# lbcb-sci/herro

Measured on NVIDIA H100. Metric: corrected_bases_per_sec, higher is better.
Workload: dtype u8 pileup/consensus + f32 forward

## Files before the change

### herro_b200/csrc/gemm_tc.cu

```cuda
#include <cstdio>
#include <cuda.h>
#include <cuda_bf16.h>

#include "common.cuh"
#include "forward.h"

namespace hb {

namespace {

constexpr int BM = 128, BN = 128, BK = 64, STAGES = 3;
constexpr int STAGE_BYTES = (2 * BM + 2 * BN) * 128;
constexpr int C_THREADS = 256, G_THREADS = 288, G_PROD_WARP = 8;

__device__ __forceinline__ uint32_t smem_u32(const void* p) { return (uint32_t)__cvta_generic_to_shared(p); }

__device__ __forceinline__ void mbar_init(uint64_t* bar, uint32_t count) {
    asm volatile("mbarrier.init.shared::cta.b64 [%0], %1;" ::"r"(smem_u32(bar)), "r"(count));
}
__device__ __forceinline__ void mbar_arrive(uint64_t* bar) {
    asm volatile("{\n\t.reg .b64 st;\n\tmbarrier.arrive.shared::cta.b64 st, [%0];\n\t}" ::"r"(smem_u32(bar)) : "memory");
}
__device__ __forceinline__ void mbar_wait(uint64_t* bar, uint32_t parity) {
    asm volatile(
// ... 141 lines not shown
}
__device__ __forceinline__ void frag_store_f32(const float (&a)[64], float* base, size_t ld, size_t row0, int c0, int fc) {
#pragma unroll
    for (int j = 0; j < 16; j++) {
        *(float2*)(base + row0 * ld + c0 + 8 * j + fc) = make_float2(a[4 * j], a[4 * j + 1]);
        *(float2*)(base + (row0 + 8) * ld + c0 + 8 * j + fc) = make_float2(a[4 * j + 2], a[4 * j + 3]);
    }
}
__device__ __forceinline__ void frag_store_split(const float (&a)[64], __nv_bfloat16* hi, __nv_bfloat16* lo, size_t ld, size_t row0, int c0,
                                                 int fc) {
#pragma unroll
    for (int j = 0; j < 16; j++) {
        uint32_t h, l;
        const size_t o0 = row0 * ld + c0 + 8 * j + fc, o1 = (row0 + 8) * ld + c0 + 8 * j + fc;
        split2(a[4 * j], a[4 * j + 1], h, l);
        *(uint32_t*)(hi + o0) = h; *(uint32_t*)(lo + o0) = l;
        split2(a[4 * j + 2], a[4 * j + 3], h, l);
        *(uint32_t*)(hi + o1) = h; *(uint32_t*)(lo + o1) = l;
    }
}
__device__ __forceinline__ void frag_store_tile(const float (&a)[64], uint8_t* tile, int r, int fc, const float* gam = nullptr,
                                                const float* bet = nullptr, const float* ln = nullptr) {
#pragma unroll
    for (int j = 0; j < 16; j++)
#pragma unroll
        for (int hf = 0; hf < 2; hf++) {
            const int rr = r + 8 * hf, c = 8 * j + fc;
            float x = a[4 * j + 2 * hf], y = a[4 * j + 2 * hf + 1];
            if (gam) {
                x = (x - ln[2 * hf]) * ln[2 * hf + 1] * gam[c] + bet[c];
                y = (y - ln[2 * hf]) * ln[2 * hf + 1] * gam[c + 1] + bet[c + 1];
            }
            uint32_t h, l;
            split2(x, y, h, l);
            const uint32_t off = (uint32_t)(j >> 3) * (2 * BM * 128) + (uint32_t)rr * 128u + (uint32_t)((((j & 7) ^ (rr & 7)) << 4) + fc * 2);
            *(uint32_t*)(tile + off) = h;
            *(uint32_t*)(tile + off + BM * 128) = l;
        }
}

}

__global__ void __launch_bounds__(G_THREADS, 1) k_gemm_ws(GemmArgs g, const __grid_constant__ CUtensorMap tmAhi,
                                                         const __grid_constant__ CUtensorMap tmAlo, const __grid_constant__ CUtensorMap tmWhi,
                                                         const __grid_constant__ CUtensorMap tmWlo) {
    extern __shared__ uint8_t smem_dyn[];
    uint8_t* smem = smem_dyn + ((1024u - (smem_u32(smem_dyn) & 1023u)) & 1023u);
    __shared__ uint64_t full_bar[STAGES], empty_bar[STAGES];
    __shared__ __align__(16) float s_lng[BN], s_lnb[BN];

    const int tid = threadIdx.x, warp = tid >> 5, lane = tid & 31;
    if (tid == 0) {
        for (int s = 0; s < STAGES; s++) { mbar_init(&full_bar[s], 1); mbar_init(&empty_bar[s], C_THREADS); }
        asm volatile("fence.mbarrier_init.release.cluster;" ::: "memory");
    }
    if (g.mode == GEMM_OUT_F32_RES_LN && tid < BN) { s_lng[tid] = g.ln_g[tid]; s_lnb[tid] = g.ln_b[tid]; }
    __syncthreads();

    const uint32_t n_items = g.m_tiles * g.n_chunks;
    const uint32_t kbs = g.k_blocks;

    if (warp == G_PROD_WARP) {
        if (lane == 0) {
            uint32_t it_stage = 0;
            for (uint32_t item = blockIdx.x; item < n_items; item += gridDim.x) {
                const int m0 = (int)((item / g.n_chunks) * BM), n0 = (int)((item % g.n_chunks) * BN);
                for (uint32_t kb = 0; kb < kbs; kb++, it_stage++) {
                    const uint32_t s = it_stage % STAGES, ph = (it_stage / STAGES) & 1;
                    mbar_wait(&empty_bar[s], ph ^ 1);
                    const uint32_t sb = smem_u32(smem + (size_t)s * STAGE_BYTES);
                    const int k0 = (int)(kb * BK);
                    mbar_arrive_expect_tx(&full_bar[s], STAGE_BYTES);
                    tma_load_2d(sb, &tmAhi, &full_bar[s], k0, m0);
                    tma_load_2d(sb + BM * 128, &tmAlo, &full_bar[s], k0, m0);
                    tma_load_2d(sb + 2 * BM * 128, &tmWhi, &full_bar[s], k0, n0);
                    tma_load_2d(sb + 2 * BM * 128 + BN * 128, &tmWlo, &full_bar[s], k0, n0);
                }
            }
        }
        return;
    }
    const int wg = warp >> 2;
    const int fr = wg * 64 + (warp & 3) * 16 + (lane >> 2), fc = (lane & 3) * 2;
    uint32_t it_stage = 0;
    float acc[64];
    for (uint32_t item = blockIdx.x; item < n_items; item += gridDim.x) {
        const uint32_t m0 = (item / g.n_chunks) * BM, n0 = (item % g.n_chunks) * BN;
        uint32_t prev = 0;
        for (uint32_t kb = 0; kb < kbs; kb++, it_stage++) {
            const uint32_t s = it_stage % STAGES, ph = (it_stage / STAGES) & 1;
            mbar_wait(&full_bar[s], ph);
            const uint32_t sb = smem_u32(smem + (size_t)s * STAGE_BYTES);
            mma_kblock(acc, sb + wg * 64 * 128, sb + BM * 128 + wg * 64 * 128, sb + 2 * BM * 128, sb + 2 * BM * 128 + BN * 128, kb == 0);
            if (kb > 0) {
                wg_wait<1>();
                mbar_arrive(&empty_bar[prev]);
            }
            prev = s;
        }
        wg_wait<0>();
        acc_fence(acc);
        mbar_arrive(&empty_bar[prev]);
        const size_t row0 = (size_t)m0 + fr;
        if (g.mode == GEMM_OUT_F32_RES_LN) {
#pragma unroll
            for (int j = 0; j < 16; j++) {
                const int c = 8 * j + fc;
                const float2 bv = *(const float2*)(g.bias + c);
                const float2 x0 = *(const float2*)(g.res + row0 * g.ldc + c), x1 = *(const float2*)(g.res + (row0 + 8) * g.ldc + c);
                acc[4 * j] = acc[4 * j] + bv.x + x0.x; acc[4 * j + 1] = acc[4 * j + 1] + bv.y + x0.y;
                acc[4 * j + 2] = acc[4 * j + 2] + bv.x + x1.x; acc[4 * j + 3] = acc[4 * j + 3] + bv.y + x1.y;
            }
            frag_store_f32(acc, g.out, g.ldc, row0, 0, fc);
            frag_layernorm(acc, s_lng, s_lnb, fc);
            frag_store_split(acc, g.out_hi, g.out_lo, g.ldo, row0, 0, fc);
            continue;
        }
#pragma unroll
        for (int j = 0; j < 16; j++) {
            const int c = (int)n0 + 8 * j + fc;
            const float2 bv = *(const float2*)(g.bias + c);
            acc[4 * j] += bv.x; acc[4 * j + 1] += bv.y; acc[4 * j + 2] += bv.x; acc[4 * j + 3] += bv.y;
            if (g.mode == GEMM_OUT_F32_RES) {
                const float2 x0 = *(const float2*)(g.res + row0 * g.ldc + c), x1 = *(const float2*)(g.res + (row0 + 8) * g.ldc + c);
                acc[4 * j] += x0.x; acc[4 * j + 1] += x0.y; acc[4 * j + 2] += x1.x; acc[4 * j + 3] += x1.y;
            } else if (g.mode == GEMM_OUT_F32_RELU || g.mode == GEMM_OUT_SPLIT_RELU) {
#pragma unroll
                for (int e = 0; e < 4; e++) acc[4 * j + e] = fmaxf(acc[4 * j + e], 0.f);
            }
        }
        if (g.mode == GEMM_OUT_SPLIT_RELU) frag_store_split(acc, g.out_hi, g.out_lo, g.ldo, row0, (int)n0, fc);
        else frag_store_f32(acc, g.out, g.ldc, row0, (int)n0, fc);
    }
}

constexpr int FFN_RING_BYTES = 2 * BN * 128;
constexpr int FFN_A_BYTES = 2 * 2 * BM * 128;
constexpr int FFN_STAGES = 4;
constexpr int FFN_THREADS = 384, FFN_PROD_WARP = 8, FFN_PROD_REGS = 24, FFN_CONS_REGS = 240;

template <int N>
__device__ __forceinline__ void ffn_retire(uint64_t* empty_bar, uint32_t it_stage) {
    wg_wait<N>();
    mbar_arrive(&empty_bar[(it_stage - 1 - N) % FFN_STAGES]);
    if constexpr (N > 0) ffn_retire<N - 1>(empty_bar, it_stage);
}

template <bool FUSE_O>
__global__ void __launch_bounds__(FFN_THREADS, 1) k_ffn_ws(FfnArgs g, const __grid_constant__ CUtensorMap tmHhi,
                                                        const __grid_constant__ CUtensorMap tmHlo, const __grid_constant__ CUtensorMap tmW1hi,
                                                        const __grid_constant__ CUtensorMap tmW1lo, const __grid_constant__ CUtensorMap tmW2hi,
                                                        const __grid_constant__ CUtensorMap tmW2lo, const __grid_constant__ CUtensorMap tmWohi,
                                                        const __grid_constant__ CUtensorMap tmWolo) {
    extern __shared__ uint8_t smem_dyn[];
    uint8_t* smem = smem_dyn + ((1024u - (smem_u32(smem_dyn) & 1023u)) & 1023u);
    uint8_t* sA1 = smem;
    uint8_t* ring = sA1 + FFN_A_BYTES;
    __shared__ uint64_t full_bar[FFN_STAGES], empty_bar[FFN_STAGES], a1_full, a1_empty;
    __shared__ __align__(16) float s_b1[512], s_b2[BN], s_lng[BN], s_lnb[BN], s_bo[BN], s_ln2g[BN], s_ln2b[BN];

    const int tid = threadIdx.x, warp = tid >> 5, lane = tid & 31;
    if (tid == 0) {
        for (int s = 0; s < FFN_STAGES; s++) { mbar_init(&full_bar[s], 1); mbar_init(&empty_bar[s], C_THREADS); }
        mbar_init(&a1_full, 1); mbar_init(&a1_empty, C_THREADS);
        asm volatile("fence.mbarrier_init.release.cluster;" ::: "memory");
    }
    for (int i = tid; i < 512; i += FFN_THREADS) s_b1[i] = g.b1[i];
    if (tid < BN) { s_b2[tid] = g.b2[tid]; s_lng[tid] = g.ln_g[tid]; s_lnb[tid] = g.ln_b[tid]; }
    if (FUSE_O && tid < BN) { s_bo[tid] = g.bo[tid]; s_ln2g[tid] = g.ln2_g[tid]; s_ln2b[tid] = g.ln2_b[tid]; }
    __syncthreads();

    if (warp >= FFN_PROD_WARP) {
        asm volatile("setmaxnreg.dec.sync.aligned.u32 %0;" ::"n"(FFN_PROD_REGS));
        if (warp == FFN_PROD_WARP && lane == 0) {
            uint32_t it_stage = 0, n_done = 0;
            auto load_w = [&](const CUtensorMap* hi, const CUtensorMap* lo, int col, int row) {
                const uint32_t s = it_stage % FFN_STAGES, ph = (it_stage / FFN_STAGES) & 1;
                mbar_wait(&empty_bar[s], ph ^ 1);
                const uint32_t sb = smem_u32(ring + (size_t)s * FFN_RING_BYTES);
                mbar_arrive_expect_tx(&full_bar[s], FFN_RING_BYTES);
                tma_load_2d(sb, hi, &full_bar[s], col, row);
                tma_load_2d(sb + BN * 128, lo, &full_bar[s], col, row);
                it_stage++;
            };
            for (uint32_t tile = blockIdx.x; tile < g.m_tiles; tile += gridDim.x, n_done++) {
                mbar_wait(&a1_empty, (n_done & 1) ^ 1);
                mbar_arrive_expect_tx(&a1_full, FFN_A_BYTES);
                for (int kb = 0; kb < 2; kb++) {
                    tma_load_2d(smem_u32(sA1) + kb * (2 * BM * 128), &tmHhi, &a1_full, kb * BK, (int)(tile * BM));
                    tma_load_2d(smem_u32(sA1) + kb * (2 * BM * 128) + BM * 128, &tmHlo, &a1_full, kb * BK, (int)(tile * BM));
                }
                if (FUSE_O)
                    for (int kb = 0; kb < 2; kb++) load_w(&tmWohi, &tmWolo, kb * BK, 0);
                for (int c = 0; c < 4; c++) {
                    for (int kb = 0; kb < 2; kb++) load_w(&tmW1hi, &tmW1lo, kb * BK, c * 128);
                    for (int kb = 0; kb < 2; kb++) load_w(&tmW2hi, &tmW2lo, c * 128 + kb * BK, 0);
                }
            }
        }
        return;
    }
    asm volatile("setmaxnreg.inc.sync.aligned.u32 %0;" ::"n"(FFN_CONS_REGS));
    const int wg = warp >> 2;
    const int fr = wg * 64 + (warp & 3) * 16 + (lane >> 2), fc = (lane & 3) * 2;
    const uint32_t a1b = smem_u32(sA1) + wg * 64 * 128;
    uint32_t it_stage = 0, n_done = 0;
    float accO[64], accF[64];
    uint32_t ahi[32], alo[32];
    auto issue = [&](float (&acc)[64], int kb, bool zero) {
        const uint32_t s = it_stage % FFN_STAGES, ph = (it_stage / FFN_STAGES) & 1;
        mbar_wait(&full_bar[s], ph);
        const uint32_t sb = smem_u32(ring + (size_t)s * FFN_RING_BYTES), a = a1b + kb * (2 * BM * 128);
        mma_kblock(acc, a, a + BM * 128, sb, sb + BN * 128, zero && kb == 0);
        it_stage++;
    };
    auto issue_f2 = [&]() {
#pragma unroll
        for (int kb = 0; kb < 2; kb++, it_stage++) {
            const uint32_t s = it_stage % FFN_STAGES, ph = (it_stage / FFN_STAGES) & 1;
            mbar_wait(&full_bar[s], ph);
            const uint32_t sb = smem_u32(ring + (size_t)s * FFN_RING_BYTES);
            mma_kblock_ra(accO, ahi, alo, kb, sb, sb + BN * 128);
        }
    };
    auto e1 = [&](int c) {
#pragma unroll
        for (int j = 0; j < 16; j++) {
            const float b0 = s_b1[c * 128 + 8 * j + fc], b1 = s_b1[c * 128 + 8 * j + fc + 1];
            split2(fmaxf(accF[4 * j] + b0, 0.f), fmaxf(accF[4 * j + 1] + b1, 0.f), ahi[2 * j], alo[2 * j]);
            split2(fmaxf(accF[4 * j + 2] + b0, 0.f), fmaxf(accF[4 * j + 3] + b1, 0.f), ahi[2 * j + 1], alo[2 * j + 1]);
        }
    };
    for (uint32_t tile = blockIdx.x; tile < g.m_tiles; tile += gridDim.x, n_done++) {
        const size_t row0 = (size_t)tile * BM + fr;
        float2 xr[32];
#pragma unroll
        for (int j = 0; j < 16; j++) {
            xr[2 * j] = *(const float2*)(g.X + row0 * BN + 8 * j + fc);
            xr[2 * j + 1] = *(const float2*)(g.X + (row0 + 8) * BN + 8 * j + fc);
        }
        if (!FUSE_O) {
#pragma unroll
            for (int j = 0; j < 16; j++) {
                const int c = 8 * j + fc;
                const float2 x0 = xr[2 * j], x1 = xr[2 * j + 1];
                accO[4 * j] = x0.x + s_b2[c]; accO[4 * j + 1] = x0.y + s_b2[c + 1];
                accO[4 * j + 2] = x1.x + s_b2[c]; accO[4 * j + 3] = x1.y + s_b2[c + 1];
            }
        }
        mbar_wait(&a1_full, n_done & 1);
        if (FUSE_O) {
            issue(accO, 0, true);
            issue(accO, 1, true);
            ffn_retire<1>(empty_bar, it_stage);
            acc_fence(accO);
#pragma unroll
            for (int j = 0; j < 16; j++) {
                const int c = 8 * j + fc;
                const float2 x0 = xr[2 * j], x1 = xr[2 * j + 1];
                accO[4 * j] = accO[4 * j] + s_bo[c] + x0.x; accO[4 * j + 1] = accO[4 * j + 1] + s_bo[c + 1] + x0.y;
                accO[4 * j + 2] = accO[4 * j + 2] + s_bo[c] + x1.x; accO[4 * j + 3] = accO[4 * j + 3] + s_bo[c + 1] + x1.y;
            }
            float ln[4];
            frag_ln_stats(accO, ln[0], ln[1], ln[2], ln[3]);
            bar_sync(1 + wg, 128);
            frag_store_tile(accO, sA1, fr, fc, s_ln2g, s_ln2b, ln);
#pragma unroll
            for (int j = 0; j < 16; j++) {
                const int c = 8 * j + fc;
                accO[4 * j] += s_b2[c]; accO[4 * j + 1] += s_b2[c + 1]; accO[4 * j + 2] += s_b2[c]; accO[4 * j + 3] += s_b2[c + 1];
            }
            fence_async_smem();
            bar_sync(1 + wg, 128);
        }
        issue(accF, 0, true);
        issue(accF, 1, true);
        ffn_retire<1>(empty_bar, it_stage);
        acc_fence(accF);
        e1(0);
        for (int c = 0; c < 3; c++) {
            issue_f2();
            issue(accF, 0, true);
            issue(accF, 1, true);
            ffn_retire<3>(empty_bar, it_stage);
            acc_fence(accF);
            reg_fence(ahi);
            reg_fence(alo);
            if (c == 2) mbar_arrive(&a1_empty);
            e1(c + 1);
        }
        issue_f2();
        ffn_retire<1>(empty_bar, it_stage);
        acc_fence(accO);
        reg_fence(ahi);
        reg_fence(alo);
        if (g.store_x) frag_store_f32(accO, g.X, BN, row0, 0, fc);
        frag_layernorm(accO, s_lng, s_lnb, fc);
        frag_store_split(accO, g.out_hi, g.out_lo, BN, row0, 0, fc);
    }
}

constexpr int QA_HROWS = 96;
constexpr int QA_RING_BYTES = 2 * QA_HROWS * 128;
constexpr int QA_STAGES = 3;
constexpr int QA_POS_BYTES = 6 * 2048;

__device__ __forceinline__ void ldsm_x4(uint32_t addr, uint32_t (&r)[4]) {
    asm volatile("ldmatrix.sync.aligned.m8n8.x4.shared.b16 {%0, %1, %2, %3}, [%4];" : "=r"(r[0]), "=r"(r[1]), "=r"(r[2]), "=r"(r[3]) : "r"(addr));
}
__device__ __forceinline__ void ldsm_x4_trans(uint32_t addr, uint32_t (&r)[4]) {
    asm volatile("ldmatrix.sync.aligned.m8n8.x4.trans.shared.b16 {%0, %1, %2, %3}, [%4];" : "=r"(r[0]), "=r"(r[1]), "=r"(r[2]), "=r"(r[3]) : "r"(addr));
}
__device__ __forceinline__ void mma16816(float (&c)[4], const uint32_t (&a)[4], uint32_t b0, uint32_t b1) {
    asm volatile("mma.sync.aligned.m16n8k16.row.col.f32.bf16.bf16.f32 {%0, %1, %2, %3}, {%4, %5, %6, %7}, {%8, %9}, {%0, %1, %2, %3};"
                 : "+f"(c[0]), "+f"(c[1]), "+f"(c[2]), "+f"(c[3])
                 : "r"(a[0]), "r"(a[1]), "r"(a[2]), "r"(a[3]), "r"(b0), "r"(b1));
}
__device__ __forceinline__ uint32_t qa_off(int row, int chunk) { return (uint32_t)(row * 64 + ((chunk ^ ((row >> 1) & 3)) << 4)); }

__global__ void __launch_bounds__(G_THREADS, 1) k_qkv_attn_ws(QkvAttnArgs g, const __grid_constant__ CUtensorMap tmHhi,
                                                             const __grid_constant__ CUtensorMap tmHlo, const __grid_constant__ CUtensorMap tmWhi,
                                                             const __grid_constant__ CUtensorMap tmWlo) {
    extern __shared__ uint8_t smem_dyn[];
    uint8_t* smem = smem_dyn + ((1024u - (smem_u32(smem_dyn) & 1023u)) & 1023u);
    uint8_t* sA = smem;
    uint8_t* ring = sA + FFN_A_BYTES;
    uint8_t* sP = ring + QA_STAGES * QA_RING_BYTES;
    __shared__ uint64_t full_bar[QA_STAGES], empty_bar[QA_STAGES], a_full, a_empty;
    __shared__ __align__(16) float s_bias[4 * QA_HROWS];

    const int tid = threadIdx.x, warp = tid >> 5, lane = tid & 31;
    if (tid == 0) {
        for (int s = 0; s < QA_STAGES; s++) { mbar_init(&full_bar[s], 1); mbar_init(&empty_bar[s], C_THREADS); }
        mbar_init(&a_full, 1); mbar_init(&a_empty, C_THREADS);
        asm volatile("fence.mbarrier_init.release.cluster;" ::: "memory");
    }
    for (int i = tid; i < 4 * QA_HROWS; i += G_THREADS) s_bias[i] = g.bias[i];
    __syncthreads();

    if (warp == G_PROD_WARP) {
        if (lane == 0) {
            uint32_t it_stage = 0, n_done = 0;
            for (uint32_t tile = blockIdx.x; tile < g.m_tiles; tile += gridDim.x, n_done++) {
                const int m0 = (int)(tile * BM);
                mbar_wait(&a_empty, (n_done & 1) ^ 1);
                mbar_arrive_expect_tx(&a_full, FFN_A_BYTES);
                for (int kb = 0; kb < 2; kb++) {
                    tma_load_2d(smem_u32(sA) + kb * (2 * BM * 128), &tmHhi, &a_full, kb * BK, m0);
                    tma_load_2d(smem_u32(sA) + kb * (2 * BM * 128) + BM * 128, &tmHlo, &a_full, kb * BK, m0);
                }
                for (int h = 0; h < 4; h++)
                    for (int kb = 0; kb < 2; kb++, it_stage++) {
                        const uint32_t s = it_stage % QA_STAGES, ph = (it_stage / QA_STAGES) & 1;
                        mbar_wait(&empty_bar[s], ph ^ 1);
                        const uint32_t sb = smem_u32(ring + (size_t)s * QA_RING_BYTES);
                        mbar_arrive_expect_tx(&full_bar[s], QA_RING_BYTES);
                        tma_load_2d(sb, &tmWhi, &full_bar[s], kb * BK, h * QA_HROWS);
                        tma_load_2d(sb + QA_HROWS * 128, &tmWlo, &full_bar[s], kb * BK, h * QA_HROWS);
                    }
            }
        }
        return;
    }
    const int wg = warp >> 2;
    const int pos = wg * 2 + ((warp & 3) >> 1);
    const int mt = warp & 1;
    const int gq = lane >> 2, tq = lane & 3;
    uint8_t* pb = sP + (size_t)pos * QA_POS_BYTES;
    uint8_t *aQh = pb, *aQl = pb + 2048, *aKh = pb + 4096, *aKl = pb + 6144, *aVh = pb + 8192, *aVl = pb + 10240;
    const uint32_t uQh = smem_u32(aQh), uQl = smem_u32(aQl), uKh = smem_u32(aKh), uKl = smem_u32(aKl), uVh = smem_u32(aVh),
                   uVl = smem_u32(aVl);
    const float scale_l2 = rsqrtf(32.f) * 1.4426950408889634f;
    const uint32_t ab = smem_u32(sA) + wg * 64 * 128;
    uint32_t it_stage = 0, n_done = 0;
    for (uint32_t tile = blockIdx.x; tile < g.m_tiles; tile += gridDim.x, n_done++) {
        mbar_wait(&a_full, n_done & 1);
        for (int h = 0; h < 4; h++) {
            float acc[48];
            for (int kb = 0; kb < 2; kb++, it_stage++) {
                const uint32_t s = it_stage % QA_STAGES, ph = (it_stage / QA_STAGES) & 1;
                mbar_wait(&full_bar[s], ph);
                const uint32_t sb = smem_u32(ring + (size_t)s * QA_RING_BYTES);
                const uint32_t a = ab + kb * (2 * BM * 128);
                const uint64_t dAh = make_desc(a), dAl = make_desc(a + BM * 128), dBh = make_desc(sb), dBl = make_desc(sb + QA_HROWS * 128);
                wg_fence();
#pragma unroll
                for (int k = 0; k < BK / 16; k++) {
                    const uint64_t adv = (uint64_t)(k * 2);
                    wgmma_n96(acc, dAh + adv, dBh + adv, (kb | k) ? 1u : 0u);
                    wgmma_n96(acc, dAl + adv, dBh + adv, 1u);
                    wgmma_n96(acc, dAh + adv, dBl + adv, 1u);
                }
                wg_commit();
            }
            wg_wait<0>();
            acc_fence(acc);
            mbar_arrive(&empty_bar[(it_stage - 2) % QA_STAGES]);
            mbar_arrive(&empty_bar[(it_stage - 1) % QA_STAGES]);
            if (h == 3) mbar_arrive(&a_empty);
            bar_sync(3 + pos, 64);
            const float* bb = s_bias + h * QA_HROWS;
#pragma unroll
            for (int j = 0; j < 12; j++) {
                const int c = 8 * j + 2 * tq;
                const float sc = j < 4 ? scale_l2 : 1.f;
                uint8_t* hi_arr = j < 4 ? aQh : (j < 8 ? aKh : aVh);
                const int cc = c & 31;
#pragma unroll
                for (int hf = 0; hf < 2; hf++) {
                    const int row = mt * 16 + hf * 8 + gq;
                    uint32_t hw, lw;
                    split2((acc[4 * j + 2 * hf] + bb[c]) * sc, (acc[4 * j + 2 * hf + 1] + bb[c + 1]) * sc, hw, lw);
                    const uint32_t off = qa_off(row, cc >> 3) + (cc & 7) * 2;
                    *(uint32_t*)(hi_arr + off) = hw;
                    *(uint32_t*)(hi_arr + 2048 + off) = lw;
                }
            }
            bar_sync(3 + pos, 64);
            float sacc[4][4];
#pragma unroll
            for (int nt = 0; nt < 4; nt++)
#pragma unroll
                for (int e = 0; e < 4; e++) sacc[nt][e] = 0.f;
            {
                uint32_t qh[2][4], ql[2][4];
#pragma unroll
                for (int ks = 0; ks < 2; ks++) {
                    const uint32_t off = qa_off(mt * 16 + (lane & 7) + ((lane >> 3) & 1) * 8, ks * 2 + (lane >> 4));
                    ldsm_x4(uQh + off, qh[ks]);
                    ldsm_x4(uQl + off, ql[ks]);
                }
#pragma unroll
                for (int ntp = 0; ntp < 2; ntp++)
#pragma unroll
                    for (int ks = 0; ks < 2; ks++) {
                        uint32_t kh[4], kl[4];
                        const uint32_t off = qa_off(ntp * 16 + (lane & 7) + (lane >> 4) * 8, ks * 2 + ((lane >> 3) & 1));
                        ldsm_x4(uKh + off, kh);
                        ldsm_x4(uKl + off, kl);
#pragma unroll
                        for (int j = 0; j < 2; j++) {
                            mma16816(sacc[ntp * 2 + j], qh[ks], kh[2 * j], kh[2 * j + 1]);
                            mma16816(sacc[ntp * 2 + j], ql[ks], kh[2 * j], kh[2 * j + 1]);
                            mma16816(sacc[ntp * 2 + j], qh[ks], kl[2 * j], kl[2 * j + 1]);
                        }
                    }
            }
            float inv[2];
#pragma unroll
            for (int hf = 0; hf < 2; hf++) {
                if (tq == 3) sacc[3][2 * hf + 1] = -INFINITY;
                float m = -INFINITY;
#pragma unroll
                for (int nt = 0; nt < 4; nt++) m = fmaxf(m, fmaxf(sacc[nt][2 * hf], sacc[nt][2 * hf + 1]));
                m = fmaxf(m, __shfl_xor_sync(HB_FULL, m, 1));
                m = fmaxf(m, __shfl_xor_sync(HB_FULL, m, 2));
                float l = 0.f;
#pragma unroll
                for (int nt = 0; nt < 4; nt++) {
                    const float p0 = exp2f(sacc[nt][2 * hf] - m), p1 = exp2f(sacc[nt][2 * hf + 1] - m);
                    sacc[nt][2 * hf] = p0; sacc[nt][2 * hf + 1] = p1;
                    l += p0 + p1;
                }
                l += __shfl_xor_sync(HB_FULL, l, 1);
                l += __shfl_xor_sync(HB_FULL, l, 2);
                const int row = mt * 16 + hf * 8 + gq;
                inv[hf] = (row < R_COLS) ? 1.f / l : 0.f;
            }
            float oacc[4][4];
#pragma unroll
            for (int dt = 0; dt < 4; dt++)
#pragma unroll
                for (int e = 0; e < 4; e++) oacc[dt][e] = 0.f;
#pragma unroll
            for (int ks = 0; ks < 2; ks++) {
                uint32_t ph[4], pl[4];
                split2(sacc[2 * ks][0], sacc[2 * ks][1], ph[0], pl[0]);
                split2(sacc[2 * ks][2], sacc[2 * ks][3], ph[1], pl[1]);
                split2(sacc[2 * ks + 1][0], sacc[2 * ks + 1][1], ph[2], pl[2]);
                split2(sacc[2 * ks + 1][2], sacc[2 * ks + 1][3], ph[3], pl[3]);
#pragma unroll
                for (int dp = 0; dp < 2; dp++) {
                    uint32_t vh[4], vl[4];
                    const uint32_t off = qa_off(ks * 16 + (lane & 7) + ((lane >> 3) & 1) * 8, dp * 2 + (lane >> 4));
                    ldsm_x4_trans(uVh + off, vh);
                    ldsm_x4_trans(uVl + off, vl);
#pragma unroll
                    for (int j = 0; j < 2; j++) {
                        mma16816(oacc[dp * 2 + j], ph, vh[2 * j], vh[2 * j + 1]);
                        mma16816(oacc[dp * 2 + j], pl, vh[2 * j], vh[2 * j + 1]);
                        mma16816(oacc[dp * 2 + j], ph, vl[2 * j], vl[2 * j + 1]);
                    }
                }
            }
            uint32_t* sth = (uint32_t*)aQh;
            uint32_t* stl = (uint32_t*)aQl;
            __syncwarp();
#pragma unroll
            for (int hf = 0; hf < 2; hf++) {
                const int row = mt * 16 + hf * 8 + gq;
#pragma unroll
                for (int dt = 0; dt < 4; dt++) {
                    uint32_t hi, lo;
                    split2(oacc[dt][2 * hf] * inv[hf], oacc[dt][2 * hf + 1] * inv[hf], hi, lo);
                    const int w = row * 16 + ((dt ^ ((row >> 1) & 3)) << 2) + tq;
                    sth[w] = hi;
                    stl[w] = lo;
                }
            }
            __syncwarp();
            const size_t rb = ((size_t)tile * BM + pos * 32) * BN + h * 32;
#pragma unroll
            for (int jj = 0; jj < 2; jj++) {
                const int rr = mt * 16 + jj * 8 + (lane >> 2), cq = lane & 3;
                const int w = rr * 16 + ((cq ^ ((rr >> 1) & 3)) << 2);
                *(uint4*)(g.out_hi + rb + (size_t)rr * BN + cq * 8) = *(const uint4*)(sth + w);
                *(uint4*)(g.out_lo + rb + (size_t)rr * BN + cq * 8) = *(const uint4*)(stl + w);
            }
            __syncwarp();
        }
    }
}

constexpr int STEM_STAGE_BYTES = (BM + 2 * BN) * 128;
constexpr int STEM_MAXK = 64;
constexpr int STEM_RP_LD = 132;
constexpr int S_PROD = 128, S_GATHER = 64, S_THREADS = 448, S_GATHER_WARP = 12;

__global__ void __launch_bounds__(S_THREADS, 1) k_stem_tc(BatchView b, StemArgs g, const __grid_constant__ CUtensorMap tmWhi,
                                                         const __grid_constant__ CUtensorMap tmWlo) {
    extern __shared__ uint8_t smem_dyn[];
    uint8_t* smem = smem_dyn + ((1024u - (smem_u32(smem_dyn) & 1023u)) & 1023u);
    uint8_t* tokbuf = smem + STAGES * STEM_STAGE_BYTES;
    uint8_t* qbuf = tokbuf + 2 * 4 * STEM_MAXK * 32;
    float* s_rp = (float*)(qbuf + 2 * 4 * STEM_MAXK * 32);
    __shared__ uint64_t full_bar[STAGES], empty_bar[STAGES], buf_full[2], buf_empty[2];
    __shared__ __align__(16) float s_bias[BN], s_lng[BN], s_lnb[BN];

    const int tid = threadIdx.x, warp = tid >> 5, lane = tid & 31;
    if (tid < BN) {
        s_bias[tid] = g.bias[tid];
        s_lng[tid] = g.out_hi ? g.ln_g[tid] : 1.f;
        s_lnb[tid] = g.out_hi ? g.ln_b[tid] : 0.f;
    }
    for (int i = tid; i < 32 * BN; i += S_THREADS) {
        const int r = i >> 7, c = i & 127;
        s_rp[r * STEM_RP_LD + c] = r < R_COLS ? g.read_pos[i] : 0.f;
    }
    if (tid == 0) {
        for (int s = 0; s < STAGES; s++) { mbar_init(&full_bar[s], S_PROD + 1); mbar_init(&empty_bar[s], C_THREADS); }
        for (int a = 0; a < 2; a++) { mbar_init(&buf_full[a], S_GATHER); mbar_init(&buf_empty[a], S_PROD); }
        asm volatile("fence.mbarrier_init.release.cluster;" ::: "memory");
    }
    __syncthreads();
    const uint32_t n_items = (g.npos + 3) / 4;
    const uint32_t kbs = g.k_blocks;
    const int K = g.taps;

    if (warp >= 8 && warp < S_GATHER_WARP) {
        const int p = tid - C_THREADS;
        const int pos = p >> 5, rd = p & 31;
        uint32_t it_stage = 0, n_done = 0;
        for (uint32_t item = blockIdx.x; item < n_items; item += gridDim.x, n_done++) {
            const uint8_t* tb = tokbuf + (n_done & 1) * 4 * STEM_MAXK * 32;
            const uint8_t* qb = qbuf + (n_done & 1) * 4 * STEM_MAXK * 32;
            mbar_wait(&buf_full[n_done & 1], (n_done >> 1) & 1);
            const uint8_t* trow = tb + pos * STEM_MAXK * 32 + rd;
            const uint8_t* qrow = qb + pos * STEM_MAXK * 32 + rd;
            for (uint32_t kb = 0; kb < kbs; kb++, it_stage++) {
                const uint32_t s = it_stage % STAGES, ph = (it_stage / STAGES) & 1;
                mbar_wait(&empty_bar[s], ph ^ 1);
                uint8_t* sA = smem + (size_t)s * STEM_STAGE_BYTES;
                if (p == 0) {
                    mbar_arrive_expect_tx(&full_bar[s], 2 * BN * 128);
                    tma_load_2d(smem_u32(sA) + BM * 128, &tmWhi, &full_bar[s], (int)(kb * BK), 0);
                    tma_load_2d(smem_u32(sA) + BM * 128 + BN * 128, &tmWlo, &full_bar[s], (int)(kb * BK), 0);
                }
                uint32_t tk[4], qq[4];
#pragma unroll
                for (int tl = 0; tl < 4; tl++) {
                    const int j = (int)kb * 4 + tl;
                    const bool in = (j < K) && (rd < R_COLS);
                    tk[tl] = in ? (uint32_t)trow[j * 32] : 0xffu;
                    qq[tl] = in ? (uint32_t)qrow[j * 32] : 0u;
                }
#pragma unroll
                for (int tl = 0; tl < 4; tl++) {
                    const uint32_t tok = tk[tl];
                    const bool live = tok < 12u;
                    const uint32_t one = (tok & 1u) ? 0x3f800000u : 0x00003f80u;
                    const uint32_t slot = tok < 11u ? (tok >> 1) : 8u;
                    uint32_t w[8];
#pragma unroll
                    for (int k = 0; k < 8; k++) w[k] = (slot == (uint32_t)k) ? one : 0u;
                    if (live) {
                        const float QS = (float)(2.0 / 93.0), QO = (float)(2.0 * 33.0 / 93.0 + 1.0);
                        const float q = __fsub_rn(__fmul_rn((float)qq[tl], QS), QO);
                        const __nv_bfloat16 qh = __float2bfloat16_rn(q);
                        const __nv_bfloat16 ql = __float2bfloat16_rn(q - __bfloat162float(qh));
                        w[5] |= (uint32_t)__bfloat16_as_ushort(qh) << 16;
                        w[6] |= (uint32_t)__bfloat16_as_ushort(ql);
                        if (tok == 11u) w[6] |= 0x3f800000u;
                    }
                    *(uint4*)(sA + (uint32_t)p * 128u + (uint32_t)(((2 * tl) ^ (p & 7)) << 4)) = make_uint4(w[0], w[1], w[2], w[3]);
                    *(uint4*)(sA + (uint32_t)p * 128u + (uint32_t)(((2 * tl + 1) ^ (p & 7)) << 4)) = make_uint4(w[4], w[5], w[6], w[7]);
                }
                fence_async_smem();
                mbar_arrive(&full_bar[s]);
            }
            mbar_arrive(&buf_empty[n_done & 1]);
        }
        return;
    }
    if (warp >= S_GATHER_WARP) {
        const int gt = tid - S_GATHER_WARP * 32;
        uint32_t n_done = 0;
        for (uint32_t item = blockIdx.x; item < n_items; item += gridDim.x, n_done++) {
            uint8_t* tb = tokbuf + (n_done & 1) * 4 * STEM_MAXK * 32;
            uint8_t* qb = qbuf + (n_done & 1) * 4 * STEM_MAXK * 32;
            uint32_t m_row = 0, m_L = 0, m_Lref = 0;
            uint64_t m_base = 0;
            if (lane < 4 && item * 4 + lane < g.npos) {
                const uint32_t w = b.fwd_win[g.n0 + item * 4 + lane];
                m_row = b.fwd_row[g.n0 + item * 4 + lane];
                m_L = b.w_L[w]; m_Lref = b.w_reflmax[w]; m_base = b.w_rowbase[w];
            }
            mbar_wait(&buf_empty[n_done & 1], ((n_done >> 1) & 1) ^ 1);
            for (int i0 = 0; i0 < 4 * K * 2; i0 += S_GATHER) {
                const int i = i0 + gt;
                const int ps = min(i / (K * 2), 3), rem = i % (K * 2), j = rem >> 1, half = rem & 1;
                const uint32_t r = __shfl_sync(HB_FULL, m_row, ps), L = __shfl_sync(HB_FULL, m_L, ps), Lref = __shfl_sync(HB_FULL, m_Lref, ps);
                const uint64_t rbase = __shfl_sync(HB_FULL, m_base, ps);
                uint4 tv = make_uint4(0xffffffffu, 0xffffffffu, 0xffffffffu, 0xffffffffu), qv = make_uint4(0, 0, 0, 0);
                const int64_t row = (int64_t)r + j - K / 2;
                if (row >= 0 && row < (int64_t)Lref) {
                    if (row < (int64_t)L) {
                        const uint64_t off = (rbase + row) * ROW_BYTES + half * 16;
                        tv = *(const uint4*)(b.mat_bases + off);
                        qv = *(const uint4*)(b.mat_quals + off);
                    } else {
                        tv = make_uint4(0x0b0b0b0bu, 0x0b0b0b0bu, 0x0b0b0b0bu, 0x0b0b0b0bu);
                        qv = make_uint4(0x7e7e7e7eu, 0x7e7e7e7eu, 0x7e7e7e7eu, 0x7e7e7e7eu);
                    }
                }
                if (i < 4 * K * 2) {
                    *(uint4*)(tb + (ps * STEM_MAXK + j) * 32 + half * 16) = tv;
                    *(uint4*)(qb + (ps * STEM_MAXK + j) * 32 + half * 16) = qv;
                }
            }
            mbar_arrive(&buf_full[n_done & 1]);
        }
        return;
    }
    const int wg = warp >> 2;
    const int fr = wg * 64 + (warp & 3) * 16 + (lane >> 2), fc = (lane & 3) * 2;
    const int rd0 = fr & 31, rd1 = (fr + 8) & 31;
    uint32_t it_stage = 0;
    float acc[64];
    for (uint32_t item = blockIdx.x; item < n_items; item += gridDim.x) {
        uint32_t prev = 0;
        for (uint32_t kb = 0; kb < kbs; kb++, it_stage++) {
            const uint32_t s = it_stage % STAGES, ph = (it_stage / STAGES) & 1;
            mbar_wait(&full_bar[s], ph);
            const uint32_t sb = smem_u32(smem + (size_t)s * STEM_STAGE_BYTES);
            const uint64_t dA = make_desc(sb + wg * 64 * 128), dBh = make_desc(sb + BM * 128), dBl = make_desc(sb + BM * 128 + BN * 128);
            wg_fence();
#pragma unroll
            for (int k = 0; k < BK / 16; k++) {
                const uint64_t adv = (uint64_t)(k * 2);
                wgmma_n128(acc, dA + adv, dBh + adv, (kb | (uint32_t)k) ? 1u : 0u);
                wgmma_n128(acc, dA + adv, dBl + adv, 1u);
            }
            wg_commit();
            if (kb > 0) {
                wg_wait<1>();
                mbar_arrive(&empty_bar[prev]);
            }
            prev = s;
        }
        wg_wait<0>();
        acc_fence(acc);
        mbar_arrive(&empty_bar[prev]);
        const size_t row0 = (size_t)item * BM + fr;
#pragma unroll
        for (int j = 0; j < 16; j++) {
            const int c = 8 * j + fc;
            const float* rp0 = s_rp + rd0 * STEM_RP_LD + c;
            const float* rp1 = s_rp + rd1 * STEM_RP_LD + c;
            acc[4 * j] = fmaxf(acc[4 * j] + s_bias[c], 0.f) + rp0[0];
            acc[4 * j + 1] = fmaxf(acc[4 * j + 1] + s_bias[c + 1], 0.f) + rp0[1];
            acc[4 * j + 2] = fmaxf(acc[4 * j + 2] + s_bias[c], 0.f) + rp1[0];
            acc[4 * j + 3] = fmaxf(acc[4 * j + 3] + s_bias[c + 1], 0.f) + rp1[1];
            if (rd0 >= R_COLS) { acc[4 * j] = 0.f; acc[4 * j + 1] = 0.f; }
            if (rd1 >= R_COLS) { acc[4 * j + 2] = 0.f; acc[4 * j + 3] = 0.f; }
        }
        frag_store_f32(acc, g.X, BN, row0, 0, fc);
        if (g.out_hi) {
            frag_layernorm(acc, s_lng, s_lnb, fc);
            frag_store_split(acc, g.out_hi, g.out_lo, BN, row0, 0, fc);
        }
    }
}

__global__ void k_split_bf16(const float* __restrict__ w, __nv_bfloat16* __restrict__ hi, __nv_bfloat16* __restrict__ lo, size_t n) {
    const size_t i = (size_t)blockIdx.x * blockDim.x + threadIdx.x;
    if (i < n) {
        const __nv_bfloat16 h = __float2bfloat16_rn(w[i]);
        hi[i] = h;
        lo[i] = __float2bfloat16_rn(w[i] - __bfloat162float(h));
    }
}

cudaError_t split_weights(const float* w, size_t n, void** hi, void** lo) {
    cudaError_t e = cudaMalloc(hi, n * 2);
    if (e != cudaSuccess) return e;
    e = cudaMalloc(lo, n * 2);
    if (e != cudaSuccess) return e;
    k_split_bf16<<<(unsigned)((n + 255) / 256), 256>>>(w, (__nv_bfloat16*)*hi, (__nv_bfloat16*)*lo, n);
    return cudaGetLastError();
}

typedef CUresult (*EncodeTiledFn)(CUtensorMap*, CUtensorMapDataType, cuuint32_t, void*, const cuuint64_t*, const cuuint64_t*,
                                  const cuuint32_t*, const cuuint32_t*, CUtensorMapInterleave, CUtensorMapSwizzle,
                                  CUtensorMapL2promotion, CUtensorMapFloatOOBfill);
static EncodeTiledFn encode_fn() {
    static EncodeTiledFn fn = nullptr;
    if (!fn) {
        void* p = nullptr;
        cudaDriverEntryPointQueryResult q;
        if (cudaGetDriverEntryPoint("cuTensorMapEncodeTiled", &p, cudaEnableDefault, &q) == cudaSuccess) fn = (EncodeTiledFn)p;
    }
    return fn;
}
static bool make_tmap(CUtensorMap* tm, const void* base, uint64_t rows, uint64_t cols, uint64_t ld, uint32_t box_rows = BM) {
    EncodeTiledFn fn = encode_fn();
    if (!fn) return false;
    const cuuint64_t gdim[2] = {cols, rows};
    const cuuint64_t gstr[1] = {ld * 2};
    const cuuint32_t box[2] = {BK, box_rows};
    const cuuint32_t estr[2] = {1, 1};
    return fn(tm, CU_TENSOR_MAP_DATA_TYPE_BFLOAT16, 2, const_cast<void*>(base), gdim, gstr, box, estr, CU_TENSOR_MAP_INTERLEAVE_NONE,
              CU_TENSOR_MAP_SWIZZLE_128B, CU_TENSOR_MAP_L2_PROMOTION_L2_128B, CU_TENSOR_MAP_FLOAT_OOB_FILL_NONE) == CUDA_SUCCESS;
}

cudaError_t gemm_tc(const GemmArgs& a, int num_sms, cudaStream_t st) {
    static bool configured = false;
    const size_t smem = (size_t)STAGES * STAGE_BYTES + 1024;
    if (!configured) {
        cudaError_t e = cudaFuncSetAttribute(k_gemm_ws, cudaFuncAttributeMaxDynamicSharedMemorySize, (int)smem);
        if (e != cudaSuccess) return e;
        configured = true;
    }
    const uint32_t items = a.m_tiles * a.n_chunks;
    if (items == 0) return cudaSuccess;
    CUtensorMap tAh, tAl, tWh, tWl;
    const uint64_t M = (uint64_t)a.m_tiles * BM, N = (uint64_t)a.n_chunks * BN;
    if (!make_tmap(&tAh, a.Ahi, M, a.K, a.lda) || !make_tmap(&tAl, a.Alo, M, a.K, a.lda) || !make_tmap(&tWh, a.Whi, N, a.K, a.K) ||
        !make_tmap(&tWl, a.Wlo, N, a.K, a.K))
        return cudaErrorInvalidValue;
    const unsigned grid = (unsigned)std::min<uint32_t>(items, (uint32_t)num_sms);
    k_gemm_ws<<<grid, G_THREADS, smem, st>>>(a, tAh, tAl, tWh, tWl);
    return cudaGetLastError();
}

cudaError_t ffn_tc(const FfnArgs& a, int num_sms, cudaStream_t st) {
    static bool configured = false;
    const size_t smem = (size_t)FFN_A_BYTES + (size_t)FFN_STAGES * FFN_RING_BYTES + 1024;
    if (!configured) {
        cudaError_t e = cudaFuncSetAttribute(k_ffn_ws<false>, cudaFuncAttributeMaxDynamicSharedMemorySize, (int)smem);
        if (e != cudaSuccess) return e;
        e = cudaFuncSetAttribute(k_ffn_ws<true>, cudaFuncAttributeMaxDynamicSharedMemorySize, (int)smem);
        if (e != cudaSuccess) return e;
        configured = true;
    }
    if (a.m_tiles == 0) return cudaSuccess;
    CUtensorMap tHh, tHl, t1h, t1l, t2h, t2l, toh, tol;
    const uint64_t T = (uint64_t)a.m_tiles * BM;
    if (!make_tmap(&tHh, a.Hhi, T, BN, BN) || !make_tmap(&tHl, a.Hlo, T, BN, BN) || !make_tmap(&t1h, a.W1hi, a.F, BN, BN) ||
        !make_tmap(&t1l, a.W1lo, a.F, BN, BN) || !make_tmap(&t2h, a.W2hi, BN, a.F, a.F) || !make_tmap(&t2l, a.W2lo, BN, a.F, a.F))
        return cudaErrorInvalidValue;
    const unsigned grid = (unsigned)std::min<uint32_t>(a.m_tiles, (uint32_t)num_sms);
    if (a.Wohi) {
        if (!make_tmap(&toh, a.Wohi, BN, BN, BN) || !make_tmap(&tol, a.Wolo, BN, BN, BN)) return cudaErrorInvalidValue;
        k_ffn_ws<true><<<grid, FFN_THREADS, smem, st>>>(a, tHh, tHl, t1h, t1l, t2h, t2l, toh, tol);
    } else {
        k_ffn_ws<false><<<grid, FFN_THREADS, smem, st>>>(a, tHh, tHl, t1h, t1l, t2h, t2l, t1h, t1l);
    }
    return cudaGetLastError();
}

cudaError_t stem_tc(const BatchView& b, const StemArgs& a, int num_sms, cudaStream_t st) {
    static bool configured = false;
    const size_t smem = (size_t)STAGES * STEM_STAGE_BYTES + 2 * 2 * 4 * STEM_MAXK * 32 + (size_t)32 * STEM_RP_LD * 4 + 1024;
    if (!configured) {
        cudaError_t e = cudaFuncSetAttribute(k_stem_tc, cudaFuncAttributeMaxDynamicSharedMemorySize, (int)smem);
        if (e != cudaSuccess) return e;
        configured = true;
    }
    const uint32_t items = (a.npos + 3) / 4;
    if (items == 0) return cudaSuccess;
    CUtensorMap tWh, tWl;
    if (!make_tmap(&tWh, a.Whi, BN, a.Kp, a.Kp) || !make_tmap(&tWl, a.Wlo, BN, a.Kp, a.Kp)) return cudaErrorInvalidValue;
    k_stem_tc<<<(unsigned)std::min<uint32_t>(items, (uint32_t)num_sms), S_THREADS, smem, st>>>(b, a, tWh, tWl);
    return cudaGetLastError();
}

cudaError_t qkv_attn_tc(const QkvAttnArgs& a, int num_sms, cudaStream_t st) {
    static bool configured = false;
    const size_t smem = (size_t)FFN_A_BYTES + (size_t)QA_STAGES * QA_RING_BYTES + (size_t)4 * QA_POS_BYTES + 1024;
    if (!configured) {
        cudaError_t e = cudaFuncSetAttribute(k_qkv_attn_ws, cudaFuncAttributeMaxDynamicSharedMemorySize, (int)smem);
        if (e != cudaSuccess) return e;
        configured = true;
    }
    if (a.m_tiles == 0) return cudaSuccess;
    CUtensorMap tHh, tHl, tWh, tWl;
    const uint64_t T = (uint64_t)a.m_tiles * BM;
    if (!make_tmap(&tHh, a.Hhi, T, BN, BN) || !make_tmap(&tHl, a.Hlo, T, BN, BN) || !make_tmap(&tWh, a.Whi, 4 * QA_HROWS, BN, BN, QA_HROWS) ||
        !make_tmap(&tWl, a.Wlo, 4 * QA_HROWS, BN, BN, QA_HROWS))
        return cudaErrorInvalidValue;
    k_qkv_attn_ws<<<(unsigned)std::min<uint32_t>(a.m_tiles, (uint32_t)num_sms), G_THREADS, smem, st>>>(a, tHh, tHl, tWh, tWl);
    return cudaGetLastError();
}

}
```

Before: 547.3 million.

## Overlap next head's QKV wgmma with attention in fused QKV-attention kernel

Restructures the fused QKV+attention kernel so the next head's projection wgmma k-blocks are issued before and during the current head's attention math, so tensor-core GEMM work overlaps softmax/mma.sync work. It also deepens the weight ring from 3 to 4 stages, grows the block to a full producer warpgroup so setmaxnreg can shift registers to the consumers, and replaces the precise reciprocal with an approximate rcp plus one Newton step. The result is more in-flight accumulator registers and more shared memory, with a risk of register spills or lower occupancy, and a slight numeric change in the softmax normalization.

```diff
diff --git a/herro_b200/csrc/gemm_tc.cu b/herro_b200/csrc/gemm_tc.cu
--- a/herro_b200/csrc/gemm_tc.cu
+++ b/herro_b200/csrc/gemm_tc.cu
@@ -467,8 +467,9 @@
 
 constexpr int QA_HROWS = 96;
 constexpr int QA_RING_BYTES = 2 * QA_HROWS * 128;
-constexpr int QA_STAGES = 3;
+constexpr int QA_STAGES = 4;
 constexpr int QA_POS_BYTES = 6 * 2048;
+constexpr int QA_THREADS = 384, QA_PROD_REGS = 24, QA_CONS_REGS = 240;
 
 __device__ __forceinline__ void ldsm_x4(uint32_t addr, uint32_t (&r)[4]) {
     asm volatile("ldmatrix.sync.aligned.m8n8.x4.shared.b16 {%0, %1, %2, %3}, [%4];" : "=r"(r[0]), "=r"(r[1]), "=r"(r[2]), "=r"(r[3]) : "r"(addr));
@@ -481,9 +482,14 @@
                  : "+f"(c[0]), "+f"(c[1]), "+f"(c[2]), "+f"(c[3])
                  : "r"(a[0]), "r"(a[1]), "r"(a[2]), "r"(a[3]), "r"(b0), "r"(b1));
 }
+__device__ __forceinline__ float rcp_normal(float x) {
+    float r;
+    asm("rcp.approx.ftz.f32 %0, %1;" : "=f"(r) : "f"(x));
+    return fmaf(r, -fmaf(x, r, -1.f), r);
+}
 __device__ __forceinline__ uint32_t qa_off(int row, int chunk) { return (uint32_t)(row * 64 + ((chunk ^ ((row >> 1) & 3)) << 4)); }
 
-__global__ void __launch_bounds__(G_THREADS, 1) k_qkv_attn_ws(QkvAttnArgs g, const __grid_constant__ CUtensorMap tmHhi,
+__global__ void __launch_bounds__(QA_THREADS, 1) k_qkv_attn_ws(QkvAttnArgs g, const __grid_constant__ CUtensorMap tmHhi,
                                                              const __grid_constant__ CUtensorMap tmHlo, const __grid_constant__ CUtensorMap tmWhi,
                                                              const __grid_constant__ CUtensorMap tmWlo) {
     extern __shared__ uint8_t smem_dyn[];
@@ -500,11 +506,12 @@
         mbar_init(&a_full, 1); mbar_init(&a_empty, C_THREADS);
         asm volatile("fence.mbarrier_init.release.cluster;" ::: "memory");
     }
-    for (int i = tid; i < 4 * QA_HROWS; i += G_THREADS) s_bias[i] = g.bias[i];
+    for (int i = tid; i < 4 * QA_HROWS; i += QA_THREADS) s_bias[i] = g.bias[i];
     __syncthreads();
 
-    if (warp == G_PROD_WARP) {
-        if (lane == 0) {
+    if (warp >= G_PROD_WARP) {
+        asm volatile("setmaxnreg.dec.sync.aligned.u32 %0;" ::"n"(QA_PROD_REGS));
+        if (warp == G_PROD_WARP && lane == 0) {
             uint32_t it_stage = 0, n_done = 0;
             for (uint32_t tile = blockIdx.x; tile < g.m_tiles; tile += gridDim.x, n_done++) {
                 const int m0 = (int)(tile * BM);
@@ -527,6 +534,7 @@
         }
         return;
     }
+    asm volatile("setmaxnreg.inc.sync.aligned.u32 %0;" ::"n"(QA_CONS_REGS));
     const int wg = warp >> 2;
     const int pos = wg * 2 + ((warp & 3) >> 1);
     const int mt = warp & 1;
@@ -538,152 +546,166 @@
     const float scale_l2 = rsqrtf(32.f) * 1.4426950408889634f;
     const uint32_t ab = smem_u32(sA) + wg * 64 * 128;
     uint32_t it_stage = 0, n_done = 0;
+    float acc[48];
+    auto issue_kblock = [&](int kb) {
+        const uint32_t s = it_stage % QA_STAGES, ph = (it_stage / QA_STAGES) & 1;
+        mbar_wait(&full_bar[s], ph);
+        const uint32_t sb = smem_u32(ring + (size_t)s * QA_RING_BYTES);
+        const uint32_t a = ab + kb * (2 * BM * 128);
+        const uint64_t dAh = make_desc(a), dAl = make_desc(a + BM * 128), dBh = make_desc(sb), dBl = make_desc(sb + QA_HROWS * 128);
+        wg_fence();
+#pragma unroll
+        for (int k = 0; k < BK / 16; k++) {
+            const uint64_t adv = (uint64_t)(k * 2);
+            wgmma_n96(acc, dAh + adv, dBh + adv, (kb | k) ? 1u : 0u);
+            wgmma_n96(acc, dAl + adv, dBh + adv, 1u);
+            wgmma_n96(acc, dAh + adv, dBl + adv, 1u);
+        }
+        wg_commit();
+        it_stage++;
+    };
+    auto drain = [&](int h) {
+        wg_wait<0>();
+        acc_fence(acc);
+        mbar_arrive(&empty_bar[(it_stage - 2) % QA_STAGES]);
+        mbar_arrive(&empty_bar[(it_stage - 1) % QA_STAGES]);
+        if (h == 3) mbar_arrive(&a_empty);
+        bar_sync(3 + pos, 64);
+        const float* bb = s_bias + h * QA_HROWS;
+#pragma unroll
+        for (int j = 0; j < 12; j++) {
+            const int c = 8 * j + 2 * tq;
+            const float sc = j < 4 ? scale_l2 : 1.f;
+            uint8_t* hi_arr = j < 4 ? aQh : (j < 8 ? aKh : aVh);
+            const int cc = c & 31;
+#pragma unroll
+            for (int hf = 0; hf < 2; hf++) {
+                const int row = mt * 16 + hf * 8 + gq;
+                uint32_t hw, lw;
+                split2((acc[4 * j + 2 * hf] + bb[c]) * sc, (acc[4 * j + 2 * hf + 1] + bb[c + 1]) * sc, hw, lw);
+                const uint32_t off = qa_off(row, cc >> 3) + (cc & 7) * 2;
+                *(uint32_t*)(hi_arr + off) = hw;
+                *(uint32_t*)(hi_arr + 2048 + off) = lw;
+            }
+        }
+    };
+    auto attend = [&](uint32_t tile, int h, bool next) {
+        float sacc[4][4];
+#pragma unroll
+        for (int nt = 0; nt < 4; nt++)
+#pragma unroll
+            for (int e = 0; e < 4; e++) sacc[nt][e] = 0.f;
+        {
+            uint32_t qh[2][4], ql[2][4];
+#pragma unroll
+            for (int ks = 0; ks < 2; ks++) {
+                const uint32_t off = qa_off(mt * 16 + (lane & 7) + ((lane >> 3) & 1) * 8, ks * 2 + (lane >> 4));
+                ldsm_x4(uQh + off, qh[ks]);
+                ldsm_x4(uQl + off, ql[ks]);
+            }
+#pragma unroll
+            for (int ntp = 0; ntp < 2; ntp++)
+#pragma unroll
+                for (int ks = 0; ks < 2; ks++) {
+                    uint32_t kh[4], kl[4];
+                    const uint32_t off = qa_off(ntp * 16 + (lane & 7) + (lane >> 4) * 8, ks * 2 + ((lane >> 3) & 1));
+                    ldsm_x4(uKh + off, kh);
+                    ldsm_x4(uKl + off, kl);
+#pragma unroll
+                    for (int j = 0; j < 2; j++) {
+                        mma16816(sacc[ntp * 2 + j], qh[ks], kh[2 * j], kh[2 * j + 1]);
+                        mma16816(sacc[ntp * 2 + j], ql[ks], kh[2 * j], kh[2 * j + 1]);
+                        mma16816(sacc[ntp * 2 + j], qh[ks], kl[2 * j], kl[2 * j + 1]);
+                    }
+                }
+        }
+        if (next) issue_kblock(1);
+        float inv[2];
+#pragma unroll
+        for (int hf = 0; hf < 2; hf++) {
+            if (tq == 3) sacc[3][2 * hf + 1] = -INFINITY;
+            float m = -INFINITY;
+#pragma unroll
+            for (int nt = 0; nt < 4; nt++) m = fmaxf(m, fmaxf(sacc[nt][2 * hf], sacc[nt][2 * hf + 1]));
+            m = fmaxf(m, __shfl_xor_sync(HB_FULL, m, 1));
+            m = fmaxf(m, __shfl_xor_sync(HB_FULL, m, 2));
+            float l = 0.f;
+#pragma unroll
+            for (int nt = 0; nt < 4; nt++) {
+                const float p0 = exp2f(sacc[nt][2 * hf] - m), p1 = exp2f(sacc[nt][2 * hf + 1] - m);
+                sacc[nt][2 * hf] = p0; sacc[nt][2 * hf + 1] = p1;
+                l += p0 + p1;
+            }
+            l += __shfl_xor_sync(HB_FULL, l, 1);
+            l += __shfl_xor_sync(HB_FULL, l, 2);
+            const int row = mt * 16 + hf * 8 + gq;
+            inv[hf] = (row < R_COLS) ? rcp_normal(l) : 0.f;
+        }
+        float oacc[4][4];
+#pragma unroll
+        for (int dt = 0; dt < 4; dt++)
+#pragma unroll
+            for (int e = 0; e < 4; e++) oacc[dt][e] = 0.f;
+#pragma unroll
+        for (int ks = 0; ks < 2; ks++) {
+            uint32_t ph[4], pl[4];
+            split2(sacc[2 * ks][0], sacc[2 * ks][1], ph[0], pl[0]);
+            split2(sacc[2 * ks][2], sacc[2 * ks][3], ph[1], pl[1]);
+            split2(sacc[2 * ks + 1][0], sacc[2 * ks + 1][1], ph[2], pl[2]);
+            split2(sacc[2 * ks + 1][2], sacc[2 * ks + 1][3], ph[3], pl[3]);
+#pragma unroll
+            for (int dp = 0; dp < 2; dp++) {
+                uint32_t vh[4], vl[4];
+                const uint32_t off = qa_off(ks * 16 + (lane & 7) + ((lane >> 3) & 1) * 8, dp * 2 + (lane >> 4));
+                ldsm_x4_trans(uVh + off, vh);
+                ldsm_x4_trans(uVl + off, vl);
+#pragma unroll
+                for (int j = 0; j < 2; j++) {
+                    mma16816(oacc[dp * 2 + j], ph, vh[2 * j], vh[2 * j + 1]);
+                    mma16816(oacc[dp * 2 + j], pl, vh[2 * j], vh[2 * j + 1]);
+                    mma16816(oacc[dp * 2 + j], ph, vl[2 * j], vl[2 * j + 1]);
+                }
+            }
+        }
+        uint32_t* sth = (uint32_t*)aQh;
+        uint32_t* stl = (uint32_t*)aQl;
+        __syncwarp();
+#pragma unroll
+        for (int hf = 0; hf < 2; hf++) {
+            const int row = mt * 16 + hf * 8 + gq;
+#pragma unroll
+            for (int dt = 0; dt < 4; dt++) {
+                uint32_t hi, lo;
+                split2(oacc[dt][2 * hf] * inv[hf], oacc[dt][2 * hf + 1] * inv[hf], hi, lo);
+                const int w = row * 16 + ((dt ^ ((row >> 1) & 3)) << 2) + tq;
+                sth[w] = hi;
+                stl[w] = lo;
+            }
+        }
+        __syncwarp();
+        const size_t rb = ((size_t)tile * BM + pos * 32) * BN + h * 32;
+#pragma unroll
+        for (int jj = 0; jj < 2; jj++) {
+            const int rr = mt * 16 + jj * 8 + (lane >> 2), cq = lane & 3;
+            const int w = rr * 16 + ((cq ^ ((rr >> 1) & 3)) << 2);
+            *(uint4*)(g.out_hi + rb + (size_t)rr * BN + cq * 8) = *(const uint4*)(sth + w);
+            *(uint4*)(g.out_lo + rb + (size_t)rr * BN + cq * 8) = *(const uint4*)(stl + w);
+        }
+        __syncwarp();
+    };
     for (uint32_t tile = blockIdx.x; tile < g.m_tiles; tile += gridDim.x, n_done++) {
         mbar_wait(&a_full, n_done & 1);
-        for (int h = 0; h < 4; h++) {
-            float acc[48];
-            for (int kb = 0; kb < 2; kb++, it_stage++) {
-                const uint32_t s = it_stage % QA_STAGES, ph = (it_stage / QA_STAGES) & 1;
-                mbar_wait(&full_bar[s], ph);
-                const uint32_t sb = smem_u32(ring + (size_t)s * QA_RING_BYTES);
-                const uint32_t a = ab + kb * (2 * BM * 128);
-                const uint64_t dAh = make_desc(a), dAl = make_desc(a + BM * 128), dBh = make_desc(sb), dBl = make_desc(sb + QA_HROWS * 128);
-                wg_fence();
-#pragma unroll
-                for (int k = 0; k < BK / 16; k++) {
-                    const uint64_t adv = (uint64_t)(k * 2);
-                    wgmma_n96(acc, dAh + adv, dBh + adv, (kb | k) ? 1u : 0u);
-                    wgmma_n96(acc, dAl + adv, dBh + adv, 1u);
-                    wgmma_n96(acc, dAh + adv, dBl + adv, 1u);
-                }
-                wg_commit();
-            }
-            wg_wait<0>();
-            acc_fence(acc);
-            mbar_arrive(&empty_bar[(it_stage - 2) % QA_STAGES]);
-            mbar_arrive(&empty_bar[(it_stage - 1) % QA_STAGES]);
-            if (h == 3) mbar_arrive(&a_empty);
+        issue_kblock(0);
+        issue_kblock(1);
+        for (int h = 0; h < 3; h++) {
+            drain(h);
+            issue_kblock(0);
             bar_sync(3 + pos, 64);
-            const float* bb = s_bias + h * QA_HROWS;
-#pragma unroll
-            for (int j = 0; j < 12; j++) {
-                const int c = 8 * j + 2 * tq;
-                const float sc = j < 4 ? scale_l2 : 1.f;
-                uint8_t* hi_arr = j < 4 ? aQh : (j < 8 ? aKh : aVh);
-                const int cc = c & 31;
-#pragma unroll
-                for (int hf = 0; hf < 2; hf++) {
-                    const int row = mt * 16 + hf * 8 + gq;
-                    uint32_t hw, lw;
-                    split2((acc[4 * j + 2 * hf] + bb[c]) * sc, (acc[4 * j + 2 * hf + 1] + bb[c + 1]) * sc, hw, lw);
-                    const uint32_t off = qa_off(row, cc >> 3) + (cc & 7) * 2;
-                    *(uint32_t*)(hi_arr + off) = hw;
-                    *(uint32_t*)(hi_arr + 2048 + off) = lw;
-                }
-            }
-            bar_sync(3 + pos, 64);
-            float sacc[4][4];
-#pragma unroll
-            for (int nt = 0; nt < 4; nt++)
-#pragma unroll
-                for (int e = 0; e < 4; e++) sacc[nt][e] = 0.f;
-            {
-                uint32_t qh[2][4], ql[2][4];
-#pragma unroll
-                for (int ks = 0; ks < 2; ks++) {
-                    const uint32_t off = qa_off(mt * 16 + (lane & 7) + ((lane >> 3) & 1) * 8, ks * 2 + (lane >> 4));
-                    ldsm_x4(uQh + off, qh[ks]);
-                    ldsm_x4(uQl + off, ql[ks]);
-                }
-#pragma unroll
-                for (int ntp = 0; ntp < 2; ntp++)
-#pragma unroll
-                    for (int ks = 0; ks < 2; ks++) {
-                        uint32_t kh[4], kl[4];
-                        const uint32_t off = qa_off(ntp * 16 + (lane & 7) + (lane >> 4) * 8, ks * 2 + ((lane >> 3) & 1));
-                        ldsm_x4(uKh + off, kh);
-                        ldsm_x4(uKl + off, kl);
-#pragma unroll
-                        for (int j = 0; j < 2; j++) {
-                            mma16816(sacc[ntp * 2 + j], qh[ks], kh[2 * j], kh[2 * j + 1]);
-                            mma16816(sacc[ntp * 2 + j], ql[ks], kh[2 * j], kh[2 * j + 1]);
-                            mma16816(sacc[ntp * 2 + j], qh[ks], kl[2 * j], kl[2 * j + 1]);
-                        }
-                    }
-            }
-            float inv[2];
-#pragma unroll
-            for (int hf = 0; hf < 2; hf++) {
-                if (tq == 3) sacc[3][2 * hf + 1] = -INFINITY;
-                float m = -INFINITY;
-#pragma unroll
-                for (int nt = 0; nt < 4; nt++) m = fmaxf(m, fmaxf(sacc[nt][2 * hf], sacc[nt][2 * hf + 1]));
-                m = fmaxf(m, __shfl_xor_sync(HB_FULL, m, 1));
-                m = fmaxf(m, __shfl_xor_sync(HB_FULL, m, 2));
-                float l = 0.f;
-#pragma unroll
-                for (int nt = 0; nt < 4; nt++) {
-                    const float p0 = exp2f(sacc[nt][2 * hf] - m), p1 = exp2f(sacc[nt][2 * hf + 1] - m);
-                    sacc[nt][2 * hf] = p0; sacc[nt][2 * hf + 1] = p1;
-                    l += p0 + p1;
-                }
-                l += __shfl_xor_sync(HB_FULL, l, 1);
-                l += __shfl_xor_sync(HB_FULL, l, 2);
-                const int row = mt * 16 + hf * 8 + gq;
-                inv[hf] = (row < R_COLS) ? 1.f / l : 0.f;
-            }
-            float oacc[4][4];
-#pragma unroll
-            for (int dt = 0; dt < 4; dt++)
-#pragma unroll
-                for (int e = 0; e < 4; e++) oacc[dt][e] = 0.f;
-#pragma unroll
-            for (int ks = 0; ks < 2; ks++) {
-                uint32_t ph[4], pl[4];
-                split2(sacc[2 * ks][0], sacc[2 * ks][1], ph[0], pl[0]);
-                split2(sacc[2 * ks][2], sacc[2 * ks][3], ph[1], pl[1]);
-                split2(sacc[2 * ks + 1][0], sacc[2 * ks + 1][1], ph[2], pl[2]);
-                split2(sacc[2 * ks + 1][2], sacc[2 * ks + 1][3], ph[3], pl[3]);
-#pragma unroll
-                for (int dp = 0; dp < 2; dp++) {
-                    uint32_t vh[4], vl[4];
-                    const uint32_t off = qa_off(ks * 16 + (lane & 7) + ((lane >> 3) & 1) * 8, dp * 2 + (lane >> 4));
-                    ldsm_x4_trans(uVh + off, vh);
-                    ldsm_x4_trans(uVl + off, vl);
-#pragma unroll
-                    for (int j = 0; j < 2; j++) {
-                        mma16816(oacc[dp * 2 + j], ph, vh[2 * j], vh[2 * j + 1]);
-                        mma16816(oacc[dp * 2 + j], pl, vh[2 * j], vh[2 * j + 1]);
-                        mma16816(oacc[dp * 2 + j], ph, vl[2 * j], vl[2 * j + 1]);
-                    }
-                }
-            }
-            uint32_t* sth = (uint32_t*)aQh;
-            uint32_t* stl = (uint32_t*)aQl;
-            __syncwarp();
-#pragma unroll
-            for (int hf = 0; hf < 2; hf++) {
-                const int row = mt * 16 + hf * 8 + gq;
-#pragma unroll
-                for (int dt = 0; dt < 4; dt++) {
-                    uint32_t hi, lo;
-                    split2(oacc[dt][2 * hf] * inv[hf], oacc[dt][2 * hf + 1] * inv[hf], hi, lo);
-                    const int w = row * 16 + ((dt ^ ((row >> 1) & 3)) << 2) + tq;
-                    sth[w] = hi;
-                    stl[w] = lo;
-                }
-            }
-            __syncwarp();
-            const size_t rb = ((size_t)tile * BM + pos * 32) * BN + h * 32;
-#pragma unroll
-            for (int jj = 0; jj < 2; jj++) {
-                const int rr = mt * 16 + jj * 8 + (lane >> 2), cq = lane & 3;
-                const int w = rr * 16 + ((cq ^ ((rr >> 1) & 3)) << 2);
-                *(uint4*)(g.out_hi + rb + (size_t)rr * BN + cq * 8) = *(const uint4*)(sth + w);
-                *(uint4*)(g.out_lo + rb + (size_t)rr * BN + cq * 8) = *(const uint4*)(stl + w);
-            }
-            __syncwarp();
-        }
+            attend(tile, h, true);
+        }
+        drain(3);
+        bar_sync(3 + pos, 64);
+        attend(tile, 3, false);
     }
 }
 
@@ -984,7 +1006,7 @@
     if (!make_tmap(&tHh, a.Hhi, T, BN, BN) || !make_tmap(&tHl, a.Hlo, T, BN, BN) || !make_tmap(&tWh, a.Whi, 4 * QA_HROWS, BN, BN, QA_HROWS) ||
         !make_tmap(&tWl, a.Wlo, 4 * QA_HROWS, BN, BN, QA_HROWS))
         return cudaErrorInvalidValue;
-    k_qkv_attn_ws<<<(unsigned)std::min<uint32_t>(a.m_tiles, (uint32_t)num_sms), G_THREADS, smem, st>>>(a, tHh, tHl, tWh, tWl);
+    k_qkv_attn_ws<<<(unsigned)std::min<uint32_t>(a.m_tiles, (uint32_t)num_sms), QA_THREADS, smem, st>>>(a, tHh, tHl, tWh, tWl);
     return cudaGetLastError();
 }
 
```

Result: faster. 555.5 million, median of 6 (+1.5%).
